# daigo0927/tf-raft

Measured on NVIDIA H100. Metric: frame-pairs/sec at 448×512 iters=12; final-flow max-abs vs ref, higher is better.
Workload: dtype f32

## Files before the change

tf_raft_b200/csrc/common.cuh:

```cuda
#pragma once
#include <cuda.h>
#include <cuda_fp16.h>
#include <cuda_runtime.h>
#include <stdint.h>

#include <type_traits>

#include "../../include/raft_b200.h"

#define RAFT_CUDA_TRY(expr)                                   \
  do {                                                        \
    cudaError_t _e = (expr);                                  \
    if (_e != cudaSuccess) return (int)_e;                    \
  } while (0)

#define RAFT_TRY(expr)                                        \
  do {                                                        \
    int _s = (expr);                                          \
    if (_s != 0) return _s;                                   \
  } while (0)

static inline int raft_launch_status() {
  cudaError_t e = cudaPeekAtLastError();
  return e == cudaSuccess ? 0 : (int)e;
// ... 150 lines not shown
        "wgmma.mma_async.sync.aligned.m64n32k16.f32.f16.f16 {%0, %1, %2, %3, %4, %5, %6, %7, %8, %9, %10, %11, %12, %13, %14, %15}, %16, %17, p, 1, 1, 0, 0;\n}\n"
        : "+f"(d[0]), "+f"(d[1]), "+f"(d[2]), "+f"(d[3]), "+f"(d[4]), "+f"(d[5]), "+f"(d[6]), "+f"(d[7]), "+f"(d[8]), "+f"(d[9]), "+f"(d[10]), "+f"(d[11]), "+f"(d[12]), "+f"(d[13]), "+f"(d[14]), "+f"(d[15])
        : "l"(a), "l"(b), "r"(scale_d));
  }
};
template <> struct Wgmma<64> {
  __device__ __forceinline__ static void mma(float (&d)[32], uint64_t a, uint64_t b, uint32_t scale_d) {
    asm volatile(
        "{\n.reg .pred p;\nsetp.ne.b32 p, %34, 0;\n"
        "wgmma.mma_async.sync.aligned.m64n64k16.f32.f16.f16 {%0, %1, %2, %3, %4, %5, %6, %7, %8, %9, %10, %11, %12, %13, %14, %15, %16, %17, %18, %19, %20, %21, %22, %23, %24, %25, %26, %27, %28, %29, %30, %31}, %32, %33, p, 1, 1, 0, 0;\n}\n"
        : "+f"(d[0]), "+f"(d[1]), "+f"(d[2]), "+f"(d[3]), "+f"(d[4]), "+f"(d[5]), "+f"(d[6]), "+f"(d[7]), "+f"(d[8]), "+f"(d[9]), "+f"(d[10]), "+f"(d[11]), "+f"(d[12]), "+f"(d[13]), "+f"(d[14]), "+f"(d[15]), "+f"(d[16]), "+f"(d[17]), "+f"(d[18]), "+f"(d[19]), "+f"(d[20]), "+f"(d[21]), "+f"(d[22]), "+f"(d[23]), "+f"(d[24]), "+f"(d[25]), "+f"(d[26]), "+f"(d[27]), "+f"(d[28]), "+f"(d[29]), "+f"(d[30]), "+f"(d[31])
        : "l"(a), "l"(b), "r"(scale_d));
  }
};
template <> struct Wgmma<96> {
  __device__ __forceinline__ static void mma(float (&d)[48], uint64_t a, uint64_t b, uint32_t scale_d) {
    asm volatile(
        "{\n.reg .pred p;\nsetp.ne.b32 p, %50, 0;\n"
        "wgmma.mma_async.sync.aligned.m64n96k16.f32.f16.f16 {%0, %1, %2, %3, %4, %5, %6, %7, %8, %9, %10, %11, %12, %13, %14, %15, %16, %17, %18, %19, %20, %21, %22, %23, %24, %25, %26, %27, %28, %29, %30, %31, %32, %33, %34, %35, %36, %37, %38, %39, %40, %41, %42, %43, %44, %45, %46, %47}, %48, %49, p, 1, 1, 0, 0;\n}\n"
        : "+f"(d[0]), "+f"(d[1]), "+f"(d[2]), "+f"(d[3]), "+f"(d[4]), "+f"(d[5]), "+f"(d[6]), "+f"(d[7]), "+f"(d[8]), "+f"(d[9]), "+f"(d[10]), "+f"(d[11]), "+f"(d[12]), "+f"(d[13]), "+f"(d[14]), "+f"(d[15]), "+f"(d[16]), "+f"(d[17]), "+f"(d[18]), "+f"(d[19]), "+f"(d[20]), "+f"(d[21]), "+f"(d[22]), "+f"(d[23]), "+f"(d[24]), "+f"(d[25]), "+f"(d[26]), "+f"(d[27]), "+f"(d[28]), "+f"(d[29]), "+f"(d[30]), "+f"(d[31]), "+f"(d[32]), "+f"(d[33]), "+f"(d[34]), "+f"(d[35]), "+f"(d[36]), "+f"(d[37]), "+f"(d[38]), "+f"(d[39]), "+f"(d[40]), "+f"(d[41]), "+f"(d[42]), "+f"(d[43]), "+f"(d[44]), "+f"(d[45]), "+f"(d[46]), "+f"(d[47])
        : "l"(a), "l"(b), "r"(scale_d));
  }
};
template <> struct Wgmma<128> {
  __device__ __forceinline__ static void mma(float (&d)[64], uint64_t a, uint64_t b, uint32_t scale_d) {
    asm volatile(
        "{\n.reg .pred p;\nsetp.ne.b32 p, %66, 0;\n"
        "wgmma.mma_async.sync.aligned.m64n128k16.f32.f16.f16 {%0, %1, %2, %3, %4, %5, %6, %7, %8, %9, %10, %11, %12, %13, %14, %15, %16, %17, %18, %19, %20, %21, %22, %23, %24, %25, %26, %27, %28, %29, %30, %31, %32, %33, %34, %35, %36, %37, %38, %39, %40, %41, %42, %43, %44, %45, %46, %47, %48, %49, %50, %51, %52, %53, %54, %55, %56, %57, %58, %59, %60, %61, %62, %63}, %64, %65, p, 1, 1, 0, 0;\n}\n"
        : "+f"(d[0]), "+f"(d[1]), "+f"(d[2]), "+f"(d[3]), "+f"(d[4]), "+f"(d[5]), "+f"(d[6]), "+f"(d[7]), "+f"(d[8]), "+f"(d[9]), "+f"(d[10]), "+f"(d[11]), "+f"(d[12]), "+f"(d[13]), "+f"(d[14]), "+f"(d[15]), "+f"(d[16]), "+f"(d[17]), "+f"(d[18]), "+f"(d[19]), "+f"(d[20]), "+f"(d[21]), "+f"(d[22]), "+f"(d[23]), "+f"(d[24]), "+f"(d[25]), "+f"(d[26]), "+f"(d[27]), "+f"(d[28]), "+f"(d[29]), "+f"(d[30]), "+f"(d[31]), "+f"(d[32]), "+f"(d[33]), "+f"(d[34]), "+f"(d[35]), "+f"(d[36]), "+f"(d[37]), "+f"(d[38]), "+f"(d[39]), "+f"(d[40]), "+f"(d[41]), "+f"(d[42]), "+f"(d[43]), "+f"(d[44]), "+f"(d[45]), "+f"(d[46]), "+f"(d[47]), "+f"(d[48]), "+f"(d[49]), "+f"(d[50]), "+f"(d[51]), "+f"(d[52]), "+f"(d[53]), "+f"(d[54]), "+f"(d[55]), "+f"(d[56]), "+f"(d[57]), "+f"(d[58]), "+f"(d[59]), "+f"(d[60]), "+f"(d[61]), "+f"(d[62]), "+f"(d[63])
        : "l"(a), "l"(b), "r"(scale_d));
  }
};

__device__ __forceinline__ void wgmma_fence() { asm volatile("wgmma.fence.sync.aligned;" ::: "memory"); }
__device__ __forceinline__ void wgmma_commit() { asm volatile("wgmma.commit_group.sync.aligned;" ::: "memory"); }
__device__ __forceinline__ void wgmma_wait_all() { asm volatile("wgmma.wait_group.sync.aligned 0;" ::: "memory"); }
template <int R>
__device__ __forceinline__ void wgmma_fence_regs(float (&d)[R]) {
#pragma unroll
  for (int i = 0; i < R; ++i) asm volatile("" : "+f"(d[i])::"memory");
}

template <int N>
__device__ __forceinline__ void wgmma_chunk3(float (&d)[N / 2], uint64_t a_hi, uint64_t a_lo, uint64_t b_hi, uint64_t b_lo,
                                             bool first) {
#pragma unroll
  for (int k = 0; k < 4; ++k) {
    Wgmma<N>::mma(d, a_hi + 2 * k, b_hi + 2 * k, (!first || k > 0) ? 1u : 0u);
    Wgmma<N>::mma(d, a_hi + 2 * k, b_lo + 2 * k, 1u);
  }
#pragma unroll
  for (int k = 0; k < 4; ++k) Wgmma<N>::mma(d, a_lo + 2 * k, b_hi + 2 * k, 1u);
}

__device__ __forceinline__ uint64_t make_desc_sw128(uint32_t smem_addr) {
  uint64_t d = 0;
  d |= (uint64_t)((smem_addr & 0x3FFFF) >> 4);
  d |= (uint64_t)1 << 16;
  d |= (uint64_t)(1024 >> 4) << 32;
  d |= (uint64_t)1 << 62;
  return d;
}

__device__ __forceinline__ void wg_sync(int wg) {
  asm volatile("bar.sync %0, 128;" ::"r"(wg + 1) : "memory");
}
#endif

}
```

tf_raft_b200/csrc/conv_tc.cuh:

```cuda
#pragma once
#include "common.cuh"
#include "kernels.cuh"
#include "tmap.cuh"

namespace raft {

enum TcEpilogue : int {
  EPI_LINEAR = 0,
  EPI_GRU_ZR = 1,
  EPI_GRU_Q = 2,
};
enum TcAct : int { ACT_NONE = 0, ACT_RELU = 1 };

constexpr int kTileM = 128;
constexpr int kChunkK = 64;
constexpr int kABytes = kTileM * kChunkK * 2;
constexpr int kMaxTileN = 128;
constexpr int kConsumerWGs = 2;
constexpr int kConsumerWarps = 4 * kConsumerWGs;
constexpr int kTcThreads = 128 * kConsumerWGs + 128;
constexpr int kStageCols = 64;
constexpr int kStagingBytes = kConsumerWGs * 64 * kStageCols * 4;
constexpr int kSmemMax = 227 * 1024;
constexpr int kSmemFixed = 1024  + kStagingBytes + 512 ;
// ... 278 lines not shown
    }
#pragma unroll
    for (int i = 0; i < N / 2; ++i) racc[i] += acc[i];
  }
}

__device__ __forceinline__ int tc_total_chunks(const TcConvParams& c) {
  return c.kh * c.kw * (c.seg_chunks[0] + (c.nseg > 1 ? c.seg_chunks[1] : 0));
}

__device__ __forceinline__ void tc_produce_tile(const TcConvParams& c, uint8_t* stages, uint64_t* full_bar, uint64_t* empty_bar,
                                                RingPos& rp, int nt, int b, int ty, int tx, unsigned int* next_item = nullptr,
                                                int* claim = nullptr) {
  const int ntaps = c.kh * c.kw;
  const int x0 = tx * c.TW * c.stride, y0 = ty * c.TH * c.stride, n0 = nt * c.bn;
  int left = tc_total_chunks(c);
  for (int tap = 0; tap < ntaps; ++tap) {
    const int dy = tap / c.kw - c.ph, dx = tap % c.kw - c.pw;
    int kc = 0;
    for (int seg = 0; seg < c.nseg; ++seg) {
      for (int ch = 0; ch < c.seg_chunks[seg]; ++ch, ++kc) {
        if (--left == 0 && claim) *claim = (int)atomicAdd(next_item, 1u);
        const RingSlot st = ring_acquire(stages, c.stage_bytes, c.nstages, full_bar, empty_bar, rp, c.stage_bytes);
        tma_load_5d(st.data, &c.a_map[seg], st.full, c.seg_c0[seg] + ch * kChunkK, x0 + dx, y0 + dy, b, 0);
        tma_load_4d(st.data + 2 * kABytes, &c.b_map, st.full, kc * kChunkK, n0, tap, 0);
      }
    }
  }
}

__device__ __forceinline__ int stg_idx(int r, int c) { return r * kStageCols + ((((c >> 2) ^ (r & 7))) << 2) + (c & 3); }

template <int N>
__device__ __forceinline__ void tc_consume_tile(const TcConvParams& c, uint8_t* stages, float* staging, uint64_t* full_bar,
                                                uint64_t* empty_bar, RingPos& rp, int wg, int tid, int nt, int b, int ty,
                                                int tx) {
  const int lane = tid & 31, w = tid >> 5;
  float racc[N / 2];
  ring_mma<N>(racc, stages, c.stage_bytes, c.nstages, full_bar, empty_bar, rp, wg, (uint32_t)(c.bn * kChunkK * 2),
              tc_total_chunks(c), c.group_chunks);

  float* stg = staging + wg * 64 * kStageCols;
  const int row = tid & 63, half = tid >> 6;
  const int m = wg * 64 + row;
  const int x = tx * c.TW + m % c.TW, y = ty * c.TH + m / c.TW;
  const bool inside = x < c.W && y < c.H;
  const size_t pix = ((size_t)b * c.H + y) * c.W + x;
  const float inv_scale = c.inv_scale ? __ldg(c.inv_scale) : 1.0f;
#pragma unroll
  for (int cb = 0; cb < (N + kStageCols - 1) / kStageCols; ++cb) {
    if (cb * kStageCols >= c.bn) break;
    wg_sync(wg);
#pragma unroll
    for (int i = cb * 8; i < min(cb * 8 + 8, N / 8); ++i) {
      const int col = 8 * (i - cb * 8) + 2 * (lane & 3), r0 = 16 * w + (lane >> 2);
      *reinterpret_cast<float2*>(stg + stg_idx(r0, col)) = make_float2(racc[4 * i], racc[4 * i + 1]);
      *reinterpret_cast<float2*>(stg + stg_idx(r0 + 8, col)) = make_float2(racc[4 * i + 2], racc[4 * i + 3]);
    }
    wg_sync(wg);
    const int c0 = cb * kStageCols + half * 32;
    if (inside && c0 < c.bn) {
      const int ncol = min(32, c.bn - c0);
      float v[32];
#pragma unroll
      for (int q = 0; q < 8; ++q) {
        const float4 t4 = *reinterpret_cast<const float4*>(stg + stg_idx(row, half * 32 + 4 * q));
        v[4 * q] = t4.x; v[4 * q + 1] = t4.y; v[4 * q + 2] = t4.z; v[4 * q + 3] = t4.w;
      }
#pragma unroll
      for (int j = 0; j < 32; ++j)
        if (j >= ncol) v[j] = 0.0f;
      if (c.mode == EPI_LINEAR) tc_epilogue_regs<EPI_LINEAR>(c, v, pix, nt * c.bn + c0, ncol, inv_scale);
      else if (c.mode == EPI_GRU_ZR) tc_epilogue_regs<EPI_GRU_ZR>(c, v, pix, nt * c.bn + c0, ncol, inv_scale);
      else tc_epilogue_regs<EPI_GRU_Q>(c, v, pix, nt * c.bn + c0, ncol, inv_scale);
    }
  }
}

template <class F>
__device__ __forceinline__ void with_mma_n(int bn, F&& f) {
  if (bn <= 16) f(std::integral_constant<int, 16>{});
  else if (bn <= 32) f(std::integral_constant<int, 32>{});
  else if (bn <= 64) f(std::integral_constant<int, 64>{});
  else if (bn <= 96) f(std::integral_constant<int, 96>{});
  else f(std::integral_constant<int, 128>{});
}

__device__ __forceinline__ void regs_producer() { asm volatile("setmaxnreg.dec.sync.aligned.u32 40;\n" ::: "memory"); }
__device__ __forceinline__ void regs_consumer() { asm volatile("setmaxnreg.inc.sync.aligned.u32 232;\n" ::: "memory"); }

__device__ __forceinline__ void tc_decode_tile(const TcConvParams& c, int t, int& nt, int& b, int& ty, int& tx) {
  const int mtiles = c.B * c.tiles_y * c.tiles_x;
  nt = t / mtiles;
  int mt = t - nt * mtiles;
  tx = mt % c.tiles_x;
  mt /= c.tiles_x;
  ty = mt % c.tiles_y;
  b = mt / c.tiles_y;
}
#endif

__global__ void __launch_bounds__(kTcThreads, 1) conv_tc_kernel(const __grid_constant__ TcConvParams p) {
#if defined(__CUDA_ARCH__)
  extern __shared__ uint8_t smem_raw[];
  uint8_t* smem = reinterpret_cast<uint8_t*>((reinterpret_cast<uintptr_t>(smem_raw) + 1023) & ~uintptr_t(1023));
  const int nst = p.nstages;
  uint8_t* stages = smem;
  float* staging = reinterpret_cast<float*>(stages + (size_t)nst * p.stage_bytes);
  uint64_t* full_bar = reinterpret_cast<uint64_t*>(reinterpret_cast<uint8_t*>(staging) + kStagingBytes);
// ... 10 lines not shown
  if (warp == kConsumerWarps && (threadIdx.x & 31) == 0) {
    prefetch_tmap(&p.a_map[0]);
    prefetch_tmap(&p.b_map);
    if (p.nseg > 1) prefetch_tmap(&p.a_map[1]);
  }
  __syncthreads();
  asm volatile("griddepcontrol.wait;" ::: "memory");
  asm volatile("griddepcontrol.launch_dependents;" ::: "memory");

  RingPos rp{0, 0u};
  if (warp >= kConsumerWarps) {
    regs_producer();
    if (warp == kConsumerWarps && elect_one()) {
      for (int t = blockIdx.x; t < ntiles; t += gridDim.x) {
        int nt, b, ty, tx;
        tc_decode_tile(p, t, nt, b, ty, tx);
        tc_produce_tile(p, stages, full_bar, empty_bar, rp, nt, b, ty, tx);
      }
    }
  } else {
    regs_consumer();
    const int wg = warp >> 2, tid = threadIdx.x & 127;
    with_mma_n(p.bn, [&](auto n) {
      for (int t = blockIdx.x; t < ntiles; t += gridDim.x) {
        int nt, b, ty, tx;
        tc_decode_tile(p, t, nt, b, ty, tx);
        tc_consume_tile<decltype(n)::value>(p, stages, staging, full_bar, empty_bar, rp, wg, tid, nt, b, ty, tx);
      }
    });
  }
#endif
}

inline void tc_pick_tile(int W, int H, int* tw, int* th) {
  long best = -1;
  for (int t = 128; t >= 8; t >>= 1) {
    const int hh = 128 / t;
    const long area = (long)round_up(W, t) * round_up(H, hh);
    if (best < 0 || area < best) {
      best = area;
      *tw = t;
      *th = hh;
    }
  }
}

inline int tc_n_split(int bn) {
  const int f = ceil_div(bn, kMaxTileN);
  return bn % (16 * f) == 0 ? f : 0;
}

inline int tc_finalize(TcConvParams& p) {
  p.tiles_x = ceil_div(p.W, p.TW);
  p.tiles_y = ceil_div(p.H, p.TH);
  p.stage_bytes = 2 * kABytes + 2 * p.bn * kChunkK * 2;
  int nst = (kSmemMax - kSmemFixed) / p.stage_bytes;
  if (nst > 8) nst = 8;
  p.nstages = nst;
  return nst * p.stage_bytes + kSmemFixed;
}

inline int tc_check(const TcConvParams& p) {
  if (p.bn % 16 != 0 || p.bn < 16 || p.bn > kMaxTileN || p.TW * p.TH != kTileM) return RAFT_ERR_BAD_SHAPE;
  if (p.mode != EPI_LINEAR && p.mode != EPI_GRU_ZR && p.mode != EPI_GRU_Q) return RAFT_ERR_UNSUPPORTED;
  if (p.group_chunks < 1) return RAFT_ERR_BAD_ARG;
  return RAFT_OK;
}

template <auto Kernel>
inline int persistent_grid(int smem, long items, unsigned* grid) {
  static int num_sms[64] = {0};
  int dev = 0;
  RAFT_CUDA_TRY(cudaGetDevice(&dev));
  int& sms = num_sms[dev & 63];
  if (!sms) {
    RAFT_CUDA_TRY(cudaFuncSetAttribute(Kernel, cudaFuncAttributeMaxDynamicSharedMemorySize, smem));
    RAFT_CUDA_TRY(cudaDeviceGetAttribute(&sms, cudaDevAttrMultiProcessorCount, dev));
  }
  *grid = (unsigned)(items < sms ? items : sms);
  return RAFT_OK;
}

inline int tc_launch(TcConvParams& p, int n_tiles_n, cudaStream_t stream) {
  RAFT_TRY(tc_check(p));
  if (p.stride < 1) p.stride = 1;
  const int smem = tc_finalize(p);
  if (p.nstages < 2) return RAFT_ERR_UNSUPPORTED;
  p.n_tiles_n = n_tiles_n;
  unsigned grid = 0;
  RAFT_TRY(persistent_grid<conv_tc_kernel>(kSmemMax, (long)p.B * p.tiles_y * p.tiles_x * n_tiles_n, &grid));
  cudaLaunchConfig_t cfg;
  memset(&cfg, 0, sizeof(cfg));
  cfg.gridDim = dim3(grid);
  cfg.blockDim = dim3((unsigned)kTcThreads);
  cfg.dynamicSmemBytes = (size_t)smem;
  cfg.stream = stream;
  cudaLaunchAttribute attr[1];
  attr[0].id = cudaLaunchAttributeProgrammaticStreamSerialization;
  attr[0].val.programmaticStreamSerializationAllowed = 1;
  cfg.attrs = attr;
  cfg.numAttrs = 1;
  ++g_launches;
  RAFT_CUDA_TRY(cudaLaunchKernelEx(&cfg, conv_tc_kernel, p));
  return raft_launch_status();
}

struct TcWeightSlot {
  size_t hi, lo, bias, scale, absmax;
  int kh, kw, cin_pad, cout_pad;
};

inline TcWeightSlot tc_weight_slot(size_t& off, int kh, int kw, int cin_pad, int cout_pad) {
  auto take = [&](size_t bytes) { const size_t o = off; off = align_up(off + bytes, 256); return o; };
  TcWeightSlot s;
  s.kh = kh; s.kw = kw; s.cin_pad = cin_pad; s.cout_pad = cout_pad;
  const size_t plane = (size_t)kh * kw * cout_pad * cin_pad * sizeof(__half);
  s.hi = take(plane);
  s.lo = take(plane);
  s.bias = take(sizeof(float) * (cout_pad + 64));
  s.scale = take(2 * sizeof(float));
  s.absmax = take(sizeof(unsigned int));
  return s;
}

struct TcCinMap { int nrange, src0[2], n[2], dst0[2]; };

inline int tc_pack_weights(uint8_t* base, const TcWeightSlot& s, const raft_conv* const src[], int nsrc,
                           const TcCinMap* cin_map, bool flatten, cudaStream_t st) {
  unsigned int* amax = reinterpret_cast<unsigned int*>(base + s.absmax);
  float* scale = reinterpret_cast<float*>(base + s.scale);
  for (int i = 0; i < nsrc; ++i) {
    const size_t nw = (size_t)src[i]->kh * src[i]->kw * src[i]->cin * src[i]->cout;
    RAFT_TRY(launch(absmax_kernel, grid_for(nw), 256, 0, st, src[i]->kernel, nw, amax));
  }
  RAFT_TRY(launch(weight_scale_kernel, 1, 1, 0, st, amax, scale));
  int cout_off = 0;
  for (int i = 0; i < nsrc; ++i) {
// ... 37 lines not shown
```

tf_raft_b200/csrc/encoder.cuh:

```cuda
#pragma once
#include <algorithm>

#include "lookup.cuh"
#include "update.cuh"

namespace raft {

enum { NORM_NONE = 0, NORM_INSTANCE = 1, NORM_BATCH = 2 };

struct EncSpec { int c0; int c[3]; int s[3]; };
inline EncSpec enc_spec(int variant) {
  if (variant == RAFT_VARIANT_BASIC) return {64, {64, 96, 128}, {1, 2, 2}};
  return {32, {32, 64, 96}, {1, 2, 2}};
}
inline int pad64(int c) { return round_up(c, 64); }

struct EncNormSlot { size_t gamma, beta, fscale, fshift; int C; };
struct EncLayout {
  TcWeightSlot conv1;
  EncNormSlot norm1;
  TcWeightSlot bc1[6], bc2[6], bds[6];
  EncNormSlot bn1[6], bn2[6], bnd[6];
  int has_ds[6], bc[6], bstride[6];
  TcWeightSlot conv2;
  size_t total;
};

inline EncLayout enc_layout(int variant, int out_dim) {
  EncLayout L;
  memset(&L, 0, sizeof(L));
  const EncSpec S = enc_spec(variant);
  size_t off = 0;
  auto take = [&](size_t bytes) { size_t o = off; off = align_up(off + bytes, 256); return o; };
  auto conv_slot = [&](int kh, int kw, int cin, int cout) { return tc_weight_slot(off, kh, kw, pad64(cin), round_up(cout, 32)); };
  auto norm_slot = [&](int C) {
    EncNormSlot n;
    n.C = C;
    n.gamma = take(sizeof(float) * (C + 64)); n.beta = take(sizeof(float) * (C + 64));
    n.fscale = take(sizeof(float) * (C + 64)); n.fshift = take(sizeof(float) * (C + 64));
// ... 97 lines not shown
    RAFT_TRY(enc_pack_norm(w->block[k].norm2, L.bn2[k], norm_type, base, st));
    if (L.has_ds[k]) {
      RAFT_TRY(enc_pack_conv(w->block[k].downsample, 1, 1, cin, c, L.bds[k], false, base, st));
      RAFT_TRY(enc_pack_norm(w->block[k].downsample_norm, L.bnd[k], norm_type, base, st));
    }
    cin = c;
  }
  RAFT_TRY(enc_pack_conv(w->conv2, 1, 1, cin, out_dim, L.conv2, false, base, st));
  return raft_launch_status();
}

struct EncCtx {
  const uint8_t* prep; EncLayout L; EncWs W; cudaStream_t st;
  int N, norm_type, stats;
  int per_image;
};

inline int enc_norm_apply(const EncCtx& c, const EncNormSlot& ns, const float* y, size_t npix, int P, int relu,
                          const float* skip32, const __half* skip_hi, const __half* skip_lo, float* out32, __half* hi,
                          __half* lo) {
  const int C = ns.C, G = c.per_image ? c.N : 1;
  const int Pg = c.per_image ? P : (int)npix;
  const float* gamma = reinterpret_cast<const float*>(c.prep + ns.gamma);
  const float* beta = reinterpret_cast<const float*>(c.prep + ns.beta);
  RAFT_TRY(launch(norm_stats_kernel, dim3((unsigned)G, kNormSplit), 256, 0, c.st, y, Pg, C, kNormSplit, c.W.part));
  RAFT_TRY(launch(norm_final_kernel, ceil_div(G * C * 32, 256), 256, 0, c.st, c.W.part, G, C, kNormSplit, gamma, 1e-3f,
                  c.W.mean, c.W.mult));
  return launch(norm_apply_kernel, grid_for(npix * (pad64(C) / 8)), 256, 0, c.st, y, npix, P, C, c.per_image, c.W.mean,
                c.W.mult, beta, relu, skip32, skip_hi, skip_lo, out32, hi, lo, pad64(C));
}

inline int enc_conv_tc(const EncCtx& c, const TcWeightSlot& cs, int cout, const EncNormSlot* ns, const __half* ahi,
                       const __half* alo, int Hin, int Win, int Hout, int Wout, int stride, int relu, const float* skip,
                       float* out32, __half* ohi, __half* olo) {
  TcConvParams p;
  memset(&p, 0, sizeof(p));
  int tw, th;
  tc_pick_tile(Wout, Hout, &tw, &th);
  if (tw * stride > 256) tw = 128 / stride, th = 128 / tw;
  const int nsplit = tc_n_split(cs.cout_pad);
  if (!nsplit) return RAFT_ERR_BAD_SHAPE;
  RAFT_TRY(make_tmap_act2(&p.a_map[0], ahi, alo, c.N, Hin, Win, cs.cin_pad, tw, th, stride));
  RAFT_TRY(tc_use_weights(p, c.prep, cs, cs.cout_pad / nsplit));
  p.nseg = 1; p.seg_chunks[0] = cs.cin_pad / kChunkK; p.seg_c0[0] = 0;
  p.stride = stride;
  if (stride == 1) { p.ph = (cs.kh - 1) / 2; p.pw = (cs.kw - 1) / 2; }
  else {
    const int tot_h = (Hout - 1) * stride + cs.kh - Hin, tot_w = (Wout - 1) * stride + cs.kw - Win;
    p.ph = (tot_h > 0 ? tot_h : 0) / 2; p.pw = (tot_w > 0 ? tot_w : 0) / 2;
  }
  p.B = c.N; p.H = Hout; p.W = Wout; p.TH = th; p.TW = tw;
  p.n_total = cout;
  p.mode = EPI_LINEAR; p.out_scale = 1.0f;
  p.out_f32 = out32; p.f32_stride = cout; p.f32_c0 = 0;
  p.out_hi = ohi; p.out_lo = olo; p.h_stride = pad64(cout); p.h_c0 = 0;
  if (ns && !c.stats && c.norm_type == NORM_BATCH) {
    p.post_scale = reinterpret_cast<const float*>(c.prep + ns->fscale);
    p.post_shift = reinterpret_cast<const float*>(c.prep + ns->fshift);
  }
  const bool fused = !(ns && c.stats);
  if (fused) {
    p.act = relu ? ACT_RELU : ACT_NONE;
    p.residual = skip; p.res_stride = cout; p.res_c0 = 0;
  } else {
    p.act = ACT_NONE; p.out_hi = nullptr; p.out_lo = nullptr;
  }
  p.group_chunks = 5;
  return tc_launch(p, nsplit, c.st);
}

inline int encoder_forward(int variant, int norm_type, int out_dim, const void* prepared, const float* images, int N,
                           int H, int W, int training, int image_norm, float* out, void* ws, size_t ws_bytes, cudaStream_t st) {
  EncCtx c;
  c.prep = reinterpret_cast<const uint8_t*>(prepared);
  c.L = enc_layout(variant, out_dim);
  c.W = enc_ws_layout(ws, variant, N, H, W);
  if (c.W.total > ws_bytes) return RAFT_ERR_WORKSPACE;
  c.st = st; c.N = N; c.norm_type = norm_type;
  c.stats = (norm_type == NORM_INSTANCE) || (norm_type == NORM_BATCH && training);
  c.per_image = norm_type == NORM_INSTANCE;
  const EncSpec S = enc_spec(variant);
  const EncLayout& L = c.L;
  const EncWs& E = c.W;

  int h = (H + 1) / 2, w = (W + 1) / 2;
  {
    const size_t npix = (size_t)N * h * w;
    const int tot_h = (h - 1) * 2 + 7 - H, tot_w = (w - 1) * 2 + 7 - W;
    const float* src = images;
    if (image_norm) {
      const size_t nimg = (size_t)N * H * W * 3;
      RAFT_TRY(launch(image_norm_kernel, grid_for(nimg), 256, 0, st, images, E.O32, nimg));
      src = E.O32;
    }
    RAFT_TRY(launch(stem_im2col_kernel, grid_for(npix * 24), 256, 0, st, src, N, H, W, h, w, (tot_h > 0 ? tot_h : 0) / 2,
                    (tot_w > 0 ? tot_w : 0) / 2, 0, E.Ih, E.Il));
    if (!c.stats && pad64(S.c0) != S.c0) {
      RAFT_CUDA_TRY(cudaMemsetAsync(E.Xh, 0, npix * pad64(S.c0) * 2, st));
      RAFT_CUDA_TRY(cudaMemsetAsync(E.Xl, 0, npix * pad64(S.c0) * 2, st));
    }
    RAFT_TRY(enc_conv_tc(c, L.conv1, S.c0, &L.norm1, E.Ih, E.Il, h, w, h, w, 1, 1, nullptr, c.stats ? E.Y32 : E.X32, E.Xh, E.Xl));
// ... 40 lines not shown
```

tf_raft_b200/csrc/tmap.cuh:

```cuda
#pragma once
#include <mutex>

#include "common.cuh"

namespace raft {

typedef CUresult (*EncodeTiledFn)(CUtensorMap*, CUtensorMapDataType, cuuint32_t, void*, const cuuint64_t*,
                                  const cuuint64_t*, const cuuint32_t*, const cuuint32_t*, CUtensorMapInterleave,
                                  CUtensorMapSwizzle, CUtensorMapL2promotion, CUtensorMapFloatOOBfill);

inline EncodeTiledFn encode_tiled_fn() {
  static EncodeTiledFn fn = nullptr;
  static std::once_flag once;
  std::call_once(once, [] {
    void* p = nullptr;
    cudaDriverEntryPointQueryResult q;
    if (cudaGetDriverEntryPoint("cuTensorMapEncodeTiled", &p, cudaEnableDefault, &q) == cudaSuccess &&
        q == cudaDriverEntryPointSuccess)
      fn = reinterpret_cast<EncodeTiledFn>(p);
  });
  return fn;
}

inline int make_tmap_f16(CUtensorMap* out, const void* base, int rank, const uint64_t* dims,
                         const uint64_t* strides_bytes, const uint32_t* box, const uint32_t* elem_strides = nullptr) {
  EncodeTiledFn fn = encode_tiled_fn();
  if (!fn) return RAFT_ERR_DRIVER;
  cuuint64_t gdim[5], gstr[4];
  cuuint32_t bx[5], es[5];
  for (int i = 0; i < rank; ++i) {
    gdim[i] = dims[i];
    bx[i] = box[i];
    es[i] = elem_strides ? elem_strides[i] : 1;
    if (i > 0) gstr[i - 1] = strides_bytes[i - 1];
  }
  CUresult r = fn(out, CU_TENSOR_MAP_DATA_TYPE_FLOAT16, (cuuint32_t)rank, const_cast<void*>(base), gdim, gstr, bx,
                  es, CU_TENSOR_MAP_INTERLEAVE_NONE, CU_TENSOR_MAP_SWIZZLE_128B, CU_TENSOR_MAP_L2_PROMOTION_L2_256B,
                  CU_TENSOR_MAP_FLOAT_OOB_FILL_NONE);
  return r == CUDA_SUCCESS ? 0 : RAFT_ERR_DRIVER;
}

inline int make_tmap_act2(CUtensorMap* out, const __half* hi, const __half* lo, int B, int H, int W, int cstride, int tw,
                          int th, int stride = 1) {
  const ptrdiff_t pstride = reinterpret_cast<const char*>(lo) - reinterpret_cast<const char*>(hi);
  if (pstride <= 0 || (pstride & 15)) return RAFT_ERR_BAD_ARG;
  if (tw * stride > 256 || th * stride > 256) return RAFT_ERR_BAD_SHAPE;
  uint64_t dims[5] = {(uint64_t)cstride, (uint64_t)W, (uint64_t)H, (uint64_t)B, 2};
  uint64_t str[4] = {(uint64_t)cstride * 2, (uint64_t)W * cstride * 2, (uint64_t)H * W * cstride * 2, (uint64_t)pstride};
  uint32_t box[5] = {64, (uint32_t)(tw * stride), (uint32_t)(th * stride), 1, 2};
  uint32_t es[5] = {1, (uint32_t)stride, (uint32_t)stride, 1, 1};
  return make_tmap_f16(out, hi, 5, dims, str, box, es);
}
inline int make_tmap_wgt2(CUtensorMap* out, const __half* hi, const __half* lo, int taps, int cout_pad, int cin_pad,
                          int bn) {
  const ptrdiff_t pstride = reinterpret_cast<const char*>(lo) - reinterpret_cast<const char*>(hi);
  if (pstride <= 0 || (pstride & 15)) return RAFT_ERR_BAD_ARG;
  uint64_t dims[4] = {(uint64_t)cin_pad, (uint64_t)cout_pad, (uint64_t)taps, 2};
  uint64_t str[3] = {(uint64_t)cin_pad * 2, (uint64_t)cout_pad * cin_pad * 2, (uint64_t)pstride};
  uint32_t box[4] = {64, (uint32_t)bn, 1, 2};
  return make_tmap_f16(out, hi, 4, dims, str, box);
}

}
```

Before: 312.3.

## Add row-reuse 3x3 conv kernel loading taller activation boxes once per tile

Adds a specialised tensor-core conv kernel for 3x3 stride-1 convs with a single 64-channel input chunk. It loads three column-shifted activation boxes, each three rows taller than the tile, and reuses them across the vertical taps, so activation data is no longer re-fetched for every one of the nine taps. It also keeps one wgmma group in flight before releasing a weight stage. The encoder uses this path by default when a layer is eligible. The cost is more shared memory for the activation boxes, which leaves fewer weight stages, plus new tile-selection logic.

```diff
diff --git a/tf_raft_b200/csrc/common.cuh b/tf_raft_b200/csrc/common.cuh
--- a/tf_raft_b200/csrc/common.cuh
+++ b/tf_raft_b200/csrc/common.cuh
@@ -209,6 +209,7 @@
 __device__ __forceinline__ void wgmma_fence() { asm volatile("wgmma.fence.sync.aligned;" ::: "memory"); }
 __device__ __forceinline__ void wgmma_commit() { asm volatile("wgmma.commit_group.sync.aligned;" ::: "memory"); }
 __device__ __forceinline__ void wgmma_wait_all() { asm volatile("wgmma.wait_group.sync.aligned 0;" ::: "memory"); }
+__device__ __forceinline__ void wgmma_wait_prev() { asm volatile("wgmma.wait_group.sync.aligned 1;" ::: "memory"); }
 template <int R>
 __device__ __forceinline__ void wgmma_fence_regs(float (&d)[R]) {
 #pragma unroll
diff --git a/tf_raft_b200/csrc/conv_tc.cuh b/tf_raft_b200/csrc/conv_tc.cuh
--- a/tf_raft_b200/csrc/conv_tc.cuh
+++ b/tf_raft_b200/csrc/conv_tc.cuh
@@ -334,14 +334,23 @@
 __device__ __forceinline__ int stg_idx(int r, int c) { return r * kStageCols + ((((c >> 2) ^ (r & 7))) << 2) + (c & 3); }
 
 template <int N>
+__device__ __forceinline__ void tc_store_tile(const TcConvParams& c, const float (&racc)[N / 2], float* staging, int wg,
+                                              int tid, int nt, int b, int ty, int tx);
+
+template <int N>
 __device__ __forceinline__ void tc_consume_tile(const TcConvParams& c, uint8_t* stages, float* staging, uint64_t* full_bar,
                                                 uint64_t* empty_bar, RingPos& rp, int wg, int tid, int nt, int b, int ty,
                                                 int tx) {
-  const int lane = tid & 31, w = tid >> 5;
   float racc[N / 2];
   ring_mma<N>(racc, stages, c.stage_bytes, c.nstages, full_bar, empty_bar, rp, wg, (uint32_t)(c.bn * kChunkK * 2),
               tc_total_chunks(c), c.group_chunks);
-
+  tc_store_tile<N>(c, racc, staging, wg, tid, nt, b, ty, tx);
+}
+
+template <int N>
+__device__ __forceinline__ void tc_store_tile(const TcConvParams& c, const float (&racc)[N / 2], float* staging, int wg,
+                                              int tid, int nt, int b, int ty, int tx) {
+  const int lane = tid & 31, w = tid >> 5;
   float* stg = staging + wg * 64 * kStageCols;
   const int row = tid & 63, half = tid >> 6;
   const int m = wg * 64 + row;
@@ -453,6 +462,112 @@
 #endif
 }
 
+constexpr int kRowTaps = 3;
+
+__host__ __device__ __forceinline__ int tc_rows_box_bytes(int tw, int th) { return 2 * tw * (th + kRowTaps - 1) * 128; }
+
+__global__ void __launch_bounds__(kTcThreads, 1) conv_tc_rows_kernel(const __grid_constant__ TcConvParams p) {
+#if defined(__CUDA_ARCH__)
+  extern __shared__ uint8_t smem_raw[];
+  uint8_t* smem = reinterpret_cast<uint8_t*>((reinterpret_cast<uintptr_t>(smem_raw) + 1023) & ~uintptr_t(1023));
+  const int nst = p.nstages, abytes = tc_rows_box_bytes(p.TW, p.TH);
+  uint8_t* abox = smem;
+  uint8_t* wst = abox + (size_t)kRowTaps * abytes;
+  float* staging = reinterpret_cast<float*>(wst + (size_t)nst * p.stage_bytes);
+  uint64_t* full_bar = reinterpret_cast<uint64_t*>(reinterpret_cast<uint8_t*>(staging) + kStagingBytes);
+  uint64_t* empty_bar = full_bar + nst;
+  uint64_t* afull = empty_bar + nst;
+  uint64_t* aempty = afull + kRowTaps;
+
+  const int warp = threadIdx.x >> 5;
+  const int ntiles = p.B * p.tiles_y * p.tiles_x * p.n_tiles_n;
+
+  if (threadIdx.x == 0) {
+    ring_init(full_bar, empty_bar, nst);
+    ring_init(afull, aempty, kRowTaps);
+    fence_mbar_init();
+  }
+  if (warp == kConsumerWarps && (threadIdx.x & 31) == 0) {
+    prefetch_tmap(&p.a_map[0]);
+    prefetch_tmap(&p.b_map);
+  }
+  __syncthreads();
+  asm volatile("griddepcontrol.wait;" ::: "memory");
+  asm volatile("griddepcontrol.launch_dependents;" ::: "memory");
+
+  RingPos rp{0, 0u};
+  uint32_t apar = 0;
+  if (warp >= kConsumerWarps) {
+    regs_producer();
+    if (warp == kConsumerWarps && elect_one()) {
+      for (int t = blockIdx.x; t < ntiles; t += gridDim.x, apar ^= 1u) {
+        int nt, b, ty, tx;
+        tc_decode_tile(p, t, nt, b, ty, tx);
+        const int x0 = tx * p.TW, y0 = ty * p.TH, n0 = nt * p.bn;
+        for (int tap = 0; tap < kRowTaps * kRowTaps; ++tap) {
+          if (tap < kRowTaps) {
+            mbar_wait(&aempty[tap], apar ^ 1u);
+            mbar_arrive_expect_tx(&afull[tap], (uint32_t)abytes);
+            tma_load_5d(abox + (size_t)tap * abytes, &p.a_map[0], &afull[tap], p.seg_c0[0], x0 + tap - p.pw, y0 - p.ph, b, 0);
+          }
+          const RingSlot st = ring_acquire(wst, p.stage_bytes, nst, full_bar, empty_bar, rp, p.stage_bytes);
+          tma_load_4d(st.data, &p.b_map, st.full, 0, n0, tap, 0);
+        }
+      }
+    }
+  } else {
+    regs_consumer();
+    const int wg = warp >> 2, tid = threadIdx.x & 127, lane = threadIdx.x & 31;
+    const uint32_t a0 = smem_u32(abox), plane = (uint32_t)(abytes / 2), b_lo_off = (uint32_t)(p.bn * kChunkK * 2);
+    with_mma_n(p.bn, [&](auto n) {
+      constexpr int N = decltype(n)::value;
+      for (int t = blockIdx.x; t < ntiles; t += gridDim.x, apar ^= 1u) {
+        int nt, b, ty, tx;
+        tc_decode_tile(p, t, nt, b, ty, tx);
+        float racc[N / 2], acc[N / 2];
+#pragma unroll
+        for (int i = 0; i < N / 2; ++i) acc[i] = racc[i] = 0.0f;
+        const int total = kRowTaps * kRowTaps;
+        auto release = [&](int s, int tap) {
+          __syncwarp();
+          if (lane == 0) {
+            mbar_arrive(&empty_bar[s]);
+            if (tap >= kRowTaps * (kRowTaps - 1)) mbar_arrive(&aempty[tap - kRowTaps * (kRowTaps - 1)]);
+          }
+        };
+        for (int done = 0; done < total;) {
+          const int gend = min(total, done + p.group_chunks);
+          int pend = 0;
+          for (int first = 1; done < gend; ++done, first = 0) {
+            const int ky = done / kRowTaps, kx = done - ky * kRowTaps;
+            if (ky == 0) mbar_wait(&afull[kx], apar);
+            const int s = ring_next(rp, nst);
+            mbar_wait(&full_bar[s], (rp.par >> s) & 1u);
+            rp.par ^= 1u << s;
+            const uint32_t sa = a0 + (uint32_t)(kx * abytes) + (uint32_t)(ky * p.TW + wg * 64) * 128;
+            const uint32_t sb = smem_u32(wst + (size_t)s * p.stage_bytes);
+            wgmma_fence_regs(acc);
+            wgmma_fence();
+            wgmma_chunk3<N>(acc, make_desc_sw128(sa), make_desc_sw128(sa + plane), make_desc_sw128(sb),
+                            make_desc_sw128(sb + b_lo_off), first != 0);
+            wgmma_commit();
+            wgmma_wait_prev();
+            if (!first) release(pend, done - 1);
+            pend = s;
+          }
+          wgmma_wait_all();
+          wgmma_fence_regs(acc);
+          release(pend, done - 1);
+#pragma unroll
+          for (int i = 0; i < N / 2; ++i) racc[i] += acc[i];
+        }
+        tc_store_tile<N>(p, racc, staging, wg, tid, nt, b, ty, tx);
+      }
+    });
+  }
+#endif
+}
+
 inline void tc_pick_tile(int W, int H, int* tw, int* th) {
   long best = -1;
   for (int t = 128; t >= 8; t >>= 1) {
@@ -502,14 +617,10 @@
   return RAFT_OK;
 }
 
-inline int tc_launch(TcConvParams& p, int n_tiles_n, cudaStream_t stream) {
-  RAFT_TRY(tc_check(p));
-  if (p.stride < 1) p.stride = 1;
-  const int smem = tc_finalize(p);
-  if (p.nstages < 2) return RAFT_ERR_UNSUPPORTED;
-  p.n_tiles_n = n_tiles_n;
+template <auto Kernel>
+inline int tc_launch_kernel(const TcConvParams& p, int smem, cudaStream_t stream) {
   unsigned grid = 0;
-  RAFT_TRY(persistent_grid<conv_tc_kernel>(kSmemMax, (long)p.B * p.tiles_y * p.tiles_x * n_tiles_n, &grid));
+  RAFT_TRY(persistent_grid<Kernel>(kSmemMax, (long)p.B * p.tiles_y * p.tiles_x * p.n_tiles_n, &grid));
   cudaLaunchConfig_t cfg;
   memset(&cfg, 0, sizeof(cfg));
   cfg.gridDim = dim3(grid);
@@ -522,8 +633,54 @@
   cfg.attrs = attr;
   cfg.numAttrs = 1;
   ++g_launches;
-  RAFT_CUDA_TRY(cudaLaunchKernelEx(&cfg, conv_tc_kernel, p));
+  RAFT_CUDA_TRY(cudaLaunchKernelEx(&cfg, Kernel, p));
   return raft_launch_status();
+}
+
+inline int tc_launch(TcConvParams& p, int n_tiles_n, cudaStream_t stream) {
+  RAFT_TRY(tc_check(p));
+  if (p.stride < 1) p.stride = 1;
+  const int smem = tc_finalize(p);
+  if (p.nstages < 2) return RAFT_ERR_UNSUPPORTED;
+  p.n_tiles_n = n_tiles_n;
+  return tc_launch_kernel<conv_tc_kernel>(p, smem, stream);
+}
+
+inline int tc_rows_smem(int tw, int th, int bn, int nst) {
+  return kRowTaps * tc_rows_box_bytes(tw, th) + nst * 2 * bn * kChunkK * 2 + kSmemFixed;
+}
+
+inline bool tc_pick_rows_tile(int W, int H, int bn, int* tw, int* th) {
+  long best = -1;
+  for (int t = 8; t <= 128; t <<= 1) {
+    const int hh = 128 / t;
+    if (tc_rows_smem(t, hh, bn, 2) > kSmemMax) continue;
+    const long cost = (long)tc_rows_box_bytes(t, hh) * round_up(W, t) * round_up(H, hh);
+    if (best < 0 || cost < best) {
+      best = cost;
+      *tw = t;
+      *th = hh;
+    }
+  }
+  return best >= 0;
+}
+
+inline bool tc_rows_eligible(const TcConvParams& p) {
+  return p.kh == kRowTaps && p.kw == kRowTaps && p.ph == 1 && p.pw == 1 && p.stride == 1 && p.nseg == 1 &&
+         p.seg_chunks[0] == 1;
+}
+
+inline int tc_launch_rows(TcConvParams& p, int n_tiles_n, cudaStream_t stream) {
+  RAFT_TRY(tc_check(p));
+  if (!tc_rows_eligible(p) || p.TW < 8) return RAFT_ERR_UNSUPPORTED;
+  p.tiles_x = ceil_div(p.W, p.TW);
+  p.tiles_y = ceil_div(p.H, p.TH);
+  p.stage_bytes = 2 * p.bn * kChunkK * 2;
+  p.nstages = (kSmemMax - tc_rows_smem(p.TW, p.TH, p.bn, 0)) / p.stage_bytes;
+  if (p.nstages > 8) p.nstages = 8;
+  if (p.nstages < 2) return RAFT_ERR_UNSUPPORTED;
+  p.n_tiles_n = n_tiles_n;
+  return tc_launch_kernel<conv_tc_rows_kernel>(p, tc_rows_smem(p.TW, p.TH, p.bn, p.nstages), stream);
 }
 
 struct TcWeightSlot {
diff --git a/tf_raft_b200/csrc/encoder.cuh b/tf_raft_b200/csrc/encoder.cuh
--- a/tf_raft_b200/csrc/encoder.cuh
+++ b/tf_raft_b200/csrc/encoder.cuh
@@ -168,20 +168,23 @@
 
 inline int enc_conv_tc(const EncCtx& c, const TcWeightSlot& cs, int cout, const EncNormSlot* ns, const __half* ahi,
                        const __half* alo, int Hin, int Win, int Hout, int Wout, int stride, int relu, const float* skip,
-                       float* out32, __half* ohi, __half* olo) {
+                       float* out32, __half* ohi, __half* olo, bool rows = true) {
   TcConvParams p;
   memset(&p, 0, sizeof(p));
-  int tw, th;
-  tc_pick_tile(Wout, Hout, &tw, &th);
-  if (tw * stride > 256) tw = 128 / stride, th = 128 / tw;
   const int nsplit = tc_n_split(cs.cout_pad);
   if (!nsplit) return RAFT_ERR_BAD_SHAPE;
-  RAFT_TRY(make_tmap_act2(&p.a_map[0], ahi, alo, c.N, Hin, Win, cs.cin_pad, tw, th, stride));
   RAFT_TRY(tc_use_weights(p, c.prep, cs, cs.cout_pad / nsplit));
   p.nseg = 1; p.seg_chunks[0] = cs.cin_pad / kChunkK; p.seg_c0[0] = 0;
   p.stride = stride;
   if (stride == 1) { p.ph = (cs.kh - 1) / 2; p.pw = (cs.kw - 1) / 2; }
-  else {
+  int tw, th;
+  rows = rows && tc_rows_eligible(p) && tc_pick_rows_tile(Wout, Hout, p.bn, &tw, &th);
+  if (!rows) {
+    tc_pick_tile(Wout, Hout, &tw, &th);
+    if (tw * stride > 256) tw = 128 / stride, th = 128 / tw;
+  }
+  RAFT_TRY(make_tmap_act2(&p.a_map[0], ahi, alo, c.N, Hin, Win, cs.cin_pad, tw, rows ? th + kRowTaps - 1 : th, stride));
+  if (stride != 1) {
     const int tot_h = (Hout - 1) * stride + cs.kh - Hin, tot_w = (Wout - 1) * stride + cs.kw - Win;
     p.ph = (tot_h > 0 ? tot_h : 0) / 2; p.pw = (tot_w > 0 ? tot_w : 0) / 2;
   }
@@ -202,7 +205,7 @@
     p.act = ACT_NONE; p.out_hi = nullptr; p.out_lo = nullptr;
   }
   p.group_chunks = 5;
-  return tc_launch(p, nsplit, c.st);
+  return rows ? tc_launch_rows(p, nsplit, c.st) : tc_launch(p, nsplit, c.st);
 }
 
 inline int encoder_forward(int variant, int norm_type, int out_dim, const void* prepared, const float* images, int N,
```

Measured after the change: 316.5, median of 6. 1.01x the previous value.

## Add halo-tile 3x3 conv kernel with register-sourced WGMMA for encoder

Applied to the files above, without the earlier changes.

Adds a specialized persistent kernel for 3x3 stride-1 encoder convolutions with 64 input channels. Each tile's activation halo (hi/lo fp16 planes) is loaded once via TMA, and the nine taps read shifted A fragments from it with ldmatrix, feeding register-sourced WGMMA. Previously the activation tile was re-fetched for every tap. This cuts TMA traffic and shared-memory stage usage, but applies only to narrow encoder layers, adds a new code path, and waits on each tap's MMA before moving on.

```diff
diff --git a/tf_raft_b200/csrc/common.cuh b/tf_raft_b200/csrc/common.cuh
--- a/tf_raft_b200/csrc/common.cuh
+++ b/tf_raft_b200/csrc/common.cuh
@@ -206,6 +206,33 @@
   }
 };
 
+template <int N> struct WgmmaRs;
+template <> struct WgmmaRs<32> {
+  __device__ __forceinline__ static void mma(float (&d)[16], const uint32_t (&a)[4], uint64_t b, uint32_t scale_d) {
+    asm volatile(
+        "{\n.reg .pred p;\nsetp.ne.b32 p, %21, 0;\n"
+        "wgmma.mma_async.sync.aligned.m64n32k16.f32.f16.f16 {%0, %1, %2, %3, %4, %5, %6, %7, %8, %9, %10, %11, %12, %13, %14, %15}, {%16, %17, %18, %19}, %20, p, 1, 1, 0;\n}\n"
+        : "+f"(d[0]), "+f"(d[1]), "+f"(d[2]), "+f"(d[3]), "+f"(d[4]), "+f"(d[5]), "+f"(d[6]), "+f"(d[7]), "+f"(d[8]), "+f"(d[9]), "+f"(d[10]), "+f"(d[11]), "+f"(d[12]), "+f"(d[13]), "+f"(d[14]), "+f"(d[15])
+        : "r"(a[0]), "r"(a[1]), "r"(a[2]), "r"(a[3]), "l"(b), "r"(scale_d));
+  }
+};
+template <> struct WgmmaRs<64> {
+  __device__ __forceinline__ static void mma(float (&d)[32], const uint32_t (&a)[4], uint64_t b, uint32_t scale_d) {
+    asm volatile(
+        "{\n.reg .pred p;\nsetp.ne.b32 p, %37, 0;\n"
+        "wgmma.mma_async.sync.aligned.m64n64k16.f32.f16.f16 {%0, %1, %2, %3, %4, %5, %6, %7, %8, %9, %10, %11, %12, %13, %14, %15, %16, %17, %18, %19, %20, %21, %22, %23, %24, %25, %26, %27, %28, %29, %30, %31}, {%32, %33, %34, %35}, %36, p, 1, 1, 0;\n}\n"
+        : "+f"(d[0]), "+f"(d[1]), "+f"(d[2]), "+f"(d[3]), "+f"(d[4]), "+f"(d[5]), "+f"(d[6]), "+f"(d[7]), "+f"(d[8]), "+f"(d[9]), "+f"(d[10]), "+f"(d[11]), "+f"(d[12]), "+f"(d[13]), "+f"(d[14]), "+f"(d[15]), "+f"(d[16]), "+f"(d[17]), "+f"(d[18]), "+f"(d[19]), "+f"(d[20]), "+f"(d[21]), "+f"(d[22]), "+f"(d[23]), "+f"(d[24]), "+f"(d[25]), "+f"(d[26]), "+f"(d[27]), "+f"(d[28]), "+f"(d[29]), "+f"(d[30]), "+f"(d[31])
+        : "r"(a[0]), "r"(a[1]), "r"(a[2]), "r"(a[3]), "l"(b), "r"(scale_d));
+  }
+};
+
+__device__ __forceinline__ void ldsm_x4(uint32_t (&r)[4], uint32_t addr) {
+  asm volatile("ldmatrix.sync.aligned.m8n8.x4.shared.b16 {%0, %1, %2, %3}, [%4];"
+               : "=r"(r[0]), "=r"(r[1]), "=r"(r[2]), "=r"(r[3])
+               : "r"(addr)
+               : "memory");
+}
+
 __device__ __forceinline__ void wgmma_fence() { asm volatile("wgmma.fence.sync.aligned;" ::: "memory"); }
 __device__ __forceinline__ void wgmma_commit() { asm volatile("wgmma.commit_group.sync.aligned;" ::: "memory"); }
 __device__ __forceinline__ void wgmma_wait_all() { asm volatile("wgmma.wait_group.sync.aligned 0;" ::: "memory"); }
@@ -225,6 +252,18 @@
   }
 #pragma unroll
   for (int k = 0; k < 4; ++k) Wgmma<N>::mma(d, a_lo + 2 * k, b_hi + 2 * k, 1u);
+}
+
+template <int N>
+__device__ __forceinline__ void wgmma_chunk3_rs(float (&d)[N / 2], const uint32_t (&a_hi)[4][4], const uint32_t (&a_lo)[4][4],
+                                                uint64_t b_hi, uint64_t b_lo, bool first) {
+#pragma unroll
+  for (int k = 0; k < 4; ++k) {
+    WgmmaRs<N>::mma(d, a_hi[k], b_hi + 2 * k, (!first || k > 0) ? 1u : 0u);
+    WgmmaRs<N>::mma(d, a_hi[k], b_lo + 2 * k, 1u);
+  }
+#pragma unroll
+  for (int k = 0; k < 4; ++k) WgmmaRs<N>::mma(d, a_lo[k], b_hi + 2 * k, 1u);
 }
 
 __device__ __forceinline__ uint64_t make_desc_sw128(uint32_t smem_addr) {
diff --git a/tf_raft_b200/csrc/conv_halo.cuh b/tf_raft_b200/csrc/conv_halo.cuh
--- /dev/null
+++ b/tf_raft_b200/csrc/conv_halo.cuh
@@ -0,0 +1,172 @@
+#pragma once
+#include "conv_tc.cuh"
+
+namespace raft {
+
+constexpr int kHaloMaxPx = 34 * 6;
+constexpr int kHaloPlaneBytes = round_up(kHaloMaxPx * 128, 1024);
+constexpr int kHaloBufBytes = 2 * kHaloPlaneBytes;
+constexpr int kHaloBufs = 2;
+
+#if defined(__CUDA_ARCH__)
+template <int N>
+__device__ __forceinline__ void halo_consume_tile(const TcConvParams& c, uint8_t* halo, uint8_t* stages, float* staging,
+                                                  uint64_t* full_bar, uint64_t* empty_bar, uint64_t* hfull, uint64_t* hempty,
+                                                  RingPos& rp, RingPos& hp, int wg, int tid, int nt, int b, int ty, int tx) {
+  const int lane = tid & 31, w = tid >> 5;
+  const int m = wg * 64 + 16 * w + (lane & 7) + (lane & 8);
+  const int hx = c.TW + 2;
+  const int p0 = (m / c.TW) * hx + m % c.TW;
+  const int khalf = lane >> 4;
+
+  const int hs = ring_next(hp, kHaloBufs);
+  mbar_wait(&hfull[hs], (hp.par >> hs) & 1u);
+  hp.par ^= 1u << hs;
+  const uint32_t hbase = smem_u32(halo + (size_t)hs * kHaloBufBytes);
+  const uint32_t b_lo_off = (uint32_t)(c.bn * kChunkK * 2);
+  constexpr int kTaps = 9;
+
+  auto load_tap = [&](int t, uint32_t (&ah)[4][4], uint32_t (&al)[4][4]) {
+    const int dy = t / 3, dx = t - 3 * dy;
+    const uint32_t row = hbase + (uint32_t)(p0 + dy * hx + dx) * 128;
+    const uint32_t sw = (row >> 7) & 7;
+#pragma unroll
+    for (int k = 0; k < 4; ++k) {
+      const uint32_t a = row + (((uint32_t)(2 * k + khalf) ^ sw) << 4);
+      ldsm_x4(ah[k], a);
+      ldsm_x4(al[k], a + kHaloPlaneBytes);
+    }
+  };
+  uint32_t afr[2][2][4][4];
+  load_tap(0, afr[0][0], afr[0][1]);
+
+  float acc[N / 2], racc[N / 2];
+#pragma unroll
+  for (int i = 0; i < N / 2; ++i) acc[i] = racc[i] = 0.0f;
+#pragma unroll
+  for (int t = 0; t < kTaps; ++t) {
+    const int s = ring_next(rp, c.nstages);
+    mbar_wait(&full_bar[s], (rp.par >> s) & 1u);
+    rp.par ^= 1u << s;
+    const uint32_t sb = smem_u32(stages + (size_t)s * c.stage_bytes);
+    wgmma_fence_regs(acc);
+    wgmma_fence();
+    wgmma_chunk3_rs<N>(acc, afr[t & 1][0], afr[t & 1][1], make_desc_sw128(sb), make_desc_sw128(sb + b_lo_off),
+                       t % c.group_chunks == 0);
+    wgmma_commit();
+    if (t + 1 < kTaps) load_tap(t + 1, afr[(t + 1) & 1][0], afr[(t + 1) & 1][1]);
+    wgmma_wait_all();
+    wgmma_fence_regs(acc);
+    __syncwarp();
+    if (lane == 0) {
+      mbar_arrive(&empty_bar[s]);
+      if (t == kTaps - 1) mbar_arrive(&hempty[hs]);
+    }
+    if ((t + 1) % c.group_chunks == 0 || t == kTaps - 1) {
+#pragma unroll
+      for (int i = 0; i < N / 2; ++i) racc[i] += acc[i];
+    }
+  }
+  tc_store_tile<N>(c, staging, racc, wg, tid, nt, b, ty, tx);
+}
+#endif
+
+__global__ void __launch_bounds__(kTcThreads, 1) conv_halo_kernel(const __grid_constant__ TcConvParams p) {
+#if defined(__CUDA_ARCH__)
+  extern __shared__ uint8_t smem_raw[];
+  uint8_t* smem = reinterpret_cast<uint8_t*>((reinterpret_cast<uintptr_t>(smem_raw) + 1023) & ~uintptr_t(1023));
+  const int nst = p.nstages;
+  uint8_t* halo = smem;
+  uint8_t* stages = halo + kHaloBufs * kHaloBufBytes;
+  float* staging = reinterpret_cast<float*>(stages + (size_t)nst * p.stage_bytes);
+  uint64_t* full_bar = reinterpret_cast<uint64_t*>(reinterpret_cast<uint8_t*>(staging) + kStagingBytes);
+  uint64_t* empty_bar = full_bar + nst;
+  uint64_t* hfull = empty_bar + nst;
+  uint64_t* hempty = hfull + kHaloBufs;
+
+  const int warp = threadIdx.x >> 5;
+  const int ntiles = p.B * p.tiles_y * p.tiles_x * p.n_tiles_n;
+
+  if (threadIdx.x == 0) {
+    ring_init(full_bar, empty_bar, nst);
+    ring_init(hfull, hempty, kHaloBufs);
+    fence_mbar_init();
+  }
+  if (warp == kConsumerWarps && (threadIdx.x & 31) == 0) {
+    prefetch_tmap(&p.a_map[0]);
+    prefetch_tmap(&p.b_map);
+  }
+  __syncthreads();
+  asm volatile("griddepcontrol.wait;" ::: "memory");
+  asm volatile("griddepcontrol.launch_dependents;" ::: "memory");
+
+  RingPos rp{0, 0u}, hp{0, 0u};
+  if (warp >= kConsumerWarps) {
+    regs_producer();
+    if (warp == kConsumerWarps && elect_one()) {
+      const int halo_tx = 2 * (p.TW + 2) * (p.TH + 2) * 128;
+      const int hbytes = kHaloBufBytes, hbufs = kHaloBufs;
+      for (int t = blockIdx.x; t < ntiles; t += gridDim.x) {
+        int nt, b, ty, tx;
+        tc_decode_tile(p, t, nt, b, ty, tx);
+        const int x0 = tx * p.TW - 1, y0 = ty * p.TH - 1, n0 = nt * p.bn;
+        const RingSlot h = ring_acquire(halo, hbytes, hbufs, hfull, hempty, hp, halo_tx);
+        tma_load_5d(h.data, &p.a_map[0], h.full, 0, x0, y0, b, 0);
+        tma_load_5d(h.data + kHaloPlaneBytes, &p.a_map[0], h.full, 0, x0, y0, b, 1);
+        for (int tap = 0; tap < 9; ++tap) {
+          const RingSlot st = ring_acquire(stages, p.stage_bytes, p.nstages, full_bar, empty_bar, rp, p.stage_bytes);
+          tma_load_4d(st.data, &p.b_map, st.full, 0, n0, tap, 0);
+        }
+      }
+    }
+  } else {
+    regs_consumer();
+    const int wg = warp >> 2, tid = threadIdx.x & 127;
+    auto run = [&](auto n) {
+      for (int t = blockIdx.x; t < ntiles; t += gridDim.x) {
+        int nt, b, ty, tx;
+        tc_decode_tile(p, t, nt, b, ty, tx);
+        halo_consume_tile<decltype(n)::value>(p, halo, stages, staging, full_bar, empty_bar, hfull, hempty, rp, hp, wg, tid,
+                                              nt, b, ty, tx);
+      }
+    };
+    if (p.bn <= 32) run(std::integral_constant<int, 32>{});
+    else run(std::integral_constant<int, 64>{});
+  }
+#endif
+}
+
+inline void halo_pick_tile(int W, int H, int* tw, int* th) {
+  long best_area = -1, best_halo = 0;
+  for (int t = 32; t >= 8; t >>= 1) {
+    const int hh = 128 / t;
+    const long area = (long)round_up(W, t) * round_up(H, hh), hpx = (long)(t + 2) * (hh + 2);
+    if (best_area < 0 || area < best_area || (area == best_area && hpx < best_halo)) {
+      best_area = area;
+      best_halo = hpx;
+      *tw = t;
+      *th = hh;
+    }
+  }
+}
+
+inline bool halo_fits(const TcWeightSlot& s, int stride, int bn, int n_tiles_n) {
+  return s.kh == 3 && s.kw == 3 && stride == 1 && s.cin_pad == kChunkK && n_tiles_n == 1 && (bn == 32 || bn == 64);
+}
+
+inline int halo_launch(TcConvParams& p, cudaStream_t stream) {
+  RAFT_TRY(tc_check(p));
+  if (p.kh != 3 || p.kw != 3 || p.ph != 1 || p.pw != 1 || p.stride != 1 || p.nseg != 1 || p.seg_chunks[0] != 1 ||
+      (p.bn != 32 && p.bn != 64) || (p.TW != 8 && p.TW != 16 && p.TW != 32))
+    return RAFT_ERR_UNSUPPORTED;
+  p.tiles_x = ceil_div(p.W, p.TW);
+  p.tiles_y = ceil_div(p.H, p.TH);
+  p.n_tiles_n = 1;
+  p.stage_bytes = 2 * p.bn * kChunkK * 2;
+  const int fixed = kSmemFixed + kHaloBufs * kHaloBufBytes;
+  p.nstages = min(8, (kSmemMax - fixed) / p.stage_bytes);
+  if (p.nstages < 2) return RAFT_ERR_UNSUPPORTED;
+  return tc_launch_grid<conv_halo_kernel>(p, p.nstages * p.stage_bytes + fixed, stream);
+}
+
+}
diff --git a/tf_raft_b200/csrc/conv_tc.cuh b/tf_raft_b200/csrc/conv_tc.cuh
--- a/tf_raft_b200/csrc/conv_tc.cuh
+++ b/tf_raft_b200/csrc/conv_tc.cuh
@@ -334,14 +334,9 @@
 __device__ __forceinline__ int stg_idx(int r, int c) { return r * kStageCols + ((((c >> 2) ^ (r & 7))) << 2) + (c & 3); }
 
 template <int N>
-__device__ __forceinline__ void tc_consume_tile(const TcConvParams& c, uint8_t* stages, float* staging, uint64_t* full_bar,
-                                                uint64_t* empty_bar, RingPos& rp, int wg, int tid, int nt, int b, int ty,
-                                                int tx) {
+__device__ __forceinline__ void tc_store_tile(const TcConvParams& c, float* staging, const float (&racc)[N / 2], int wg,
+                                              int tid, int nt, int b, int ty, int tx) {
   const int lane = tid & 31, w = tid >> 5;
-  float racc[N / 2];
-  ring_mma<N>(racc, stages, c.stage_bytes, c.nstages, full_bar, empty_bar, rp, wg, (uint32_t)(c.bn * kChunkK * 2),
-              tc_total_chunks(c), c.group_chunks);
-
   float* stg = staging + wg * 64 * kStageCols;
   const int row = tid & 63, half = tid >> 6;
   const int m = wg * 64 + row;
@@ -377,6 +372,16 @@
       else tc_epilogue_regs<EPI_GRU_Q>(c, v, pix, nt * c.bn + c0, ncol, inv_scale);
     }
   }
+}
+
+template <int N>
+__device__ __forceinline__ void tc_consume_tile(const TcConvParams& c, uint8_t* stages, float* staging, uint64_t* full_bar,
+                                                uint64_t* empty_bar, RingPos& rp, int wg, int tid, int nt, int b, int ty,
+                                                int tx) {
+  float racc[N / 2];
+  ring_mma<N>(racc, stages, c.stage_bytes, c.nstages, full_bar, empty_bar, rp, wg, (uint32_t)(c.bn * kChunkK * 2),
+              tc_total_chunks(c), c.group_chunks);
+  tc_store_tile<N>(c, staging, racc, wg, tid, nt, b, ty, tx);
 }
 
 template <class F>
@@ -502,14 +507,10 @@
   return RAFT_OK;
 }
 
-inline int tc_launch(TcConvParams& p, int n_tiles_n, cudaStream_t stream) {
-  RAFT_TRY(tc_check(p));
-  if (p.stride < 1) p.stride = 1;
-  const int smem = tc_finalize(p);
-  if (p.nstages < 2) return RAFT_ERR_UNSUPPORTED;
-  p.n_tiles_n = n_tiles_n;
+template <auto Kernel>
+inline int tc_launch_grid(const TcConvParams& p, int smem, cudaStream_t stream) {
   unsigned grid = 0;
-  RAFT_TRY(persistent_grid<conv_tc_kernel>(kSmemMax, (long)p.B * p.tiles_y * p.tiles_x * n_tiles_n, &grid));
+  RAFT_TRY(persistent_grid<Kernel>(kSmemMax, (long)p.B * p.tiles_y * p.tiles_x * p.n_tiles_n, &grid));
   cudaLaunchConfig_t cfg;
   memset(&cfg, 0, sizeof(cfg));
   cfg.gridDim = dim3(grid);
@@ -522,8 +523,17 @@
   cfg.attrs = attr;
   cfg.numAttrs = 1;
   ++g_launches;
-  RAFT_CUDA_TRY(cudaLaunchKernelEx(&cfg, conv_tc_kernel, p));
+  RAFT_CUDA_TRY(cudaLaunchKernelEx(&cfg, Kernel, p));
   return raft_launch_status();
+}
+
+inline int tc_launch(TcConvParams& p, int n_tiles_n, cudaStream_t stream) {
+  RAFT_TRY(tc_check(p));
+  if (p.stride < 1) p.stride = 1;
+  const int smem = tc_finalize(p);
+  if (p.nstages < 2) return RAFT_ERR_UNSUPPORTED;
+  p.n_tiles_n = n_tiles_n;
+  return tc_launch_grid<conv_tc_kernel>(p, smem, stream);
 }
 
 struct TcWeightSlot {
diff --git a/tf_raft_b200/csrc/encoder.cuh b/tf_raft_b200/csrc/encoder.cuh
--- a/tf_raft_b200/csrc/encoder.cuh
+++ b/tf_raft_b200/csrc/encoder.cuh
@@ -1,10 +1,16 @@
 #pragma once
 #include <algorithm>
 
+#include "conv_halo.cuh"
 #include "lookup.cuh"
 #include "update.cuh"
 
 namespace raft {
+
+inline bool enc_halo_enabled() {
+  static const bool v = [] { const char* e = getenv("RAFT_B200_ENC_HALO"); return e ? atoi(e) != 0 : true; }();
+  return v;
+}
 
 enum { NORM_NONE = 0, NORM_INSTANCE = 1, NORM_BATCH = 2 };
 
@@ -172,11 +178,17 @@
   TcConvParams p;
   memset(&p, 0, sizeof(p));
   int tw, th;
-  tc_pick_tile(Wout, Hout, &tw, &th);
-  if (tw * stride > 256) tw = 128 / stride, th = 128 / tw;
   const int nsplit = tc_n_split(cs.cout_pad);
   if (!nsplit) return RAFT_ERR_BAD_SHAPE;
-  RAFT_TRY(make_tmap_act2(&p.a_map[0], ahi, alo, c.N, Hin, Win, cs.cin_pad, tw, th, stride));
+  const bool halo = enc_halo_enabled() && halo_fits(cs, stride, cs.cout_pad / nsplit, nsplit);
+  if (halo) {
+    halo_pick_tile(Wout, Hout, &tw, &th);
+    RAFT_TRY(make_tmap_halo(&p.a_map[0], ahi, alo, c.N, Hin, Win, cs.cin_pad, tw, th));
+  } else {
+    tc_pick_tile(Wout, Hout, &tw, &th);
+    if (tw * stride > 256) tw = 128 / stride, th = 128 / tw;
+    RAFT_TRY(make_tmap_act2(&p.a_map[0], ahi, alo, c.N, Hin, Win, cs.cin_pad, tw, th, stride));
+  }
   RAFT_TRY(tc_use_weights(p, c.prep, cs, cs.cout_pad / nsplit));
   p.nseg = 1; p.seg_chunks[0] = cs.cin_pad / kChunkK; p.seg_c0[0] = 0;
   p.stride = stride;
@@ -202,7 +214,7 @@
     p.act = ACT_NONE; p.out_hi = nullptr; p.out_lo = nullptr;
   }
   p.group_chunks = 5;
-  return tc_launch(p, nsplit, c.st);
+  return halo ? halo_launch(p, c.st) : tc_launch(p, nsplit, c.st);
 }
 
 inline int encoder_forward(int variant, int norm_type, int out_dim, const void* prepared, const float* images, int N,
diff --git a/tf_raft_b200/csrc/tmap.cuh b/tf_raft_b200/csrc/tmap.cuh
--- a/tf_raft_b200/csrc/tmap.cuh
+++ b/tf_raft_b200/csrc/tmap.cuh
@@ -51,6 +51,16 @@
   uint32_t es[5] = {1, (uint32_t)stride, (uint32_t)stride, 1, 1};
   return make_tmap_f16(out, hi, 5, dims, str, box, es);
 }
+inline int make_tmap_halo(CUtensorMap* out, const __half* hi, const __half* lo, int B, int H, int W, int cstride, int tw,
+                          int th) {
+  const ptrdiff_t pstride = reinterpret_cast<const char*>(lo) - reinterpret_cast<const char*>(hi);
+  if (pstride <= 0 || (pstride & 15)) return RAFT_ERR_BAD_ARG;
+  if (tw + 2 > 256 || th + 2 > 256) return RAFT_ERR_BAD_SHAPE;
+  uint64_t dims[5] = {(uint64_t)cstride, (uint64_t)W, (uint64_t)H, (uint64_t)B, 2};
+  uint64_t str[4] = {(uint64_t)cstride * 2, (uint64_t)W * cstride * 2, (uint64_t)H * W * cstride * 2, (uint64_t)pstride};
+  uint32_t box[5] = {64, (uint32_t)(tw + 2), (uint32_t)(th + 2), 1, 1};
+  return make_tmap_f16(out, hi, 5, dims, str, box);
+}
 inline int make_tmap_wgt2(CUtensorMap* out, const __half* hi, const __half* lo, int taps, int cout_pad, int cin_pad,
                           int bn) {
   const ptrdiff_t pstride = reinterpret_cast<const char*>(lo) - reinterpret_cast<const char*>(hi);
```

Result: faster. 311.2 before, 315.1 after (median of 6 runs) (+1.3%).
